# yahoo/TensorFlowOnSpark

Measured on AMD Instinct MI355X. Metric: images/sec (whole node) ResNet-50 sync-SGD InputMode.SPARK, higher is better.
Workload: dtype bf16; 1 GPU; model=resnet50, global_batch=1024, per_gpu_batch=1024, parallelism=dp1

## Files before the change

### csrc/bindings.cpp

```cpp
#include <torch/extension.h>
#include <c10/hip/HIPStream.h>
#include <hip/hip_runtime.h>
#include <climits>

extern "C" {
int tfosr_bn_fast_blocks(long, int, int, int);
void tfosr_bn_apply_dual(const void*, const void*, void*, unsigned char*,
                         const float*, const float*, const float*, const float*,
                         const float*, const float*, const float*, const float*,
                         int, long, int, hipStream_t);
void tfosr_bn_bwd_stats_dual(const void*, const void*, const void*,
                             const unsigned char*, const float*, const float*,
                             const float*, const float*, float*, int, int, long,
                             int, hipStream_t);
void tfosr_bn_bwd_merge_dual(const float*, int, float*, float*, float*, float*,
                             int, hipStream_t);
void tfosr_bn_bwd_dx_dual(const void*, const void*, const void*,
                          const unsigned char*, void*, void*, const float*,
                          const float*, const float*, const float*, const float*,
                          const float*, const float*, const float*, const float*,
                          int, long, int, hipStream_t);
void tfosr_bn_stats(const void*, int, int, float*, int, int, int, long, hipStream_t);
void tfosr_bn_finalize(const float*, int, const void*, int, int, long,
                       float*, float*, float*, float*,
                       long, int, float, float, hipStream_t);
void tfosr_bn_apply(const void*, const void*, void*, unsigned char*,
// ... 58 lines not shown
                           int, hipStream_t);
int tfosr_bn_tile_ws_rows(int);
void tfosr_bn_tile_finalize(const float*, int, int, float*, float*, float*,
                            float*, float*, long, int, float, float,
                            hipStream_t);
}

namespace tfosr {
uint32_t crc32c(const uint8_t*, size_t, uint32_t);
struct ScanResult {
  std::string buffer;
  std::vector<std::pair<size_t, size_t>> records;
};
ScanResult scan_file(const std::string&, bool);
void write_file(const std::string&, const std::vector<std::string>&, bool);
}

namespace {

hipStream_t cur_stream() {
  return c10::hip::getCurrentHIPStream().stream();
}

struct BNLayout {
  bool nhwc;
  int N, C;
  long HW;
};

BNLayout bn_layout(const at::Tensor& x) {
  TORCH_CHECK(x.dim() == 4, "expected 4-D NCHW tensor");
  BNLayout l;
  l.N = x.size(0);
  l.C = x.size(1);
  l.HW = (long)x.size(2) * x.size(3);
  if (x.is_contiguous(at::MemoryFormat::ChannelsLast)) {
    l.nhwc = true;
  } else {
    TORCH_CHECK(x.is_contiguous(), "input must be contiguous (NCHW or channels_last)");
    l.nhwc = false;
  }
  return l;
}

int dtype_flag(const at::Tensor& x) {
  TORCH_CHECK(x.is_cuda(), "bn: input must be a GPU tensor");
// ... 794 lines not shown
              "conv_mfma: filter dilation fd > 1 requires input dilation "
              "D == 1");
  TORCH_CHECK(fd <= kMaxTapReach && fd * (fh - 1) <= kMaxTapReach &&
                  fd * (fw - 1) <= kMaxTapReach,
              "conv_mfma: fd, fd*(fh-1) and fd*(fw-1) must be <= ",
              kMaxTapReach);
  long taps = fh * fw;
  int N = x.size(0), Cin = x.size(1), H = x.size(2), W = x.size(3);
  TORCH_CHECK(Cin % 32 == 0, "conv_mfma requires Cin % 32 == 0");
  TORCH_CHECK(wk.size(1) == taps * Cin);
  if (OH < 0) {
    long HV = (H - 1) * D + 1, WV = (W - 1) * D + 1;
    long nh = HV + 2 * P - fd * (fh - 1) - 1;
    long nw = WV + 2 * P - fd * (fw - 1) - 1;
    TORCH_CHECK(nh >= 0 && nw >= 0,
                "conv_mfma: the dilated filter does not fit the padded "
                "input");
    OH = nh / S + 1;
    OW = nw / S + 1;
  }
  auto y = at::empty({N, Cout, OH, OW},
                     x.options().dtype(out_f32 ? at::kFloat : at::kBFloat16),
                     at::MemoryFormat::ChannelsLast);
  auto guard = at::zeros({64}, x.options());
  if (stats && D == 1 && !out_f32) {
    TORCH_CHECK(x.is_cuda() && wk.device() == x.device(),
                "conv_mfma_stats: x and wk must be on one GPU");
    const long M = (long)N * OH * OW;
    auto part = at::empty({(M + 255) / 256, 2, Cout},
                          x.options().dtype(at::kFloat));
    tfosr_conv_mfma_stats(x.data_ptr(), wk.contiguous().data_ptr(),
                          guard.data_ptr(), y.data_ptr(),
                          part.data_ptr<float>(), N, H, W, Cin, Cout, OH, OW, S,
                          P, taps, fw, (int)fd, cur_stream());
    return {y, part};
  }
  tfosr_conv_mfma(x.data_ptr(), wk.contiguous().data_ptr(), guard.data_ptr(),
                  y.data_ptr(), out_f32 ? 0 : 1, N, H, W, Cin,
                  Cout, OH, OW, S, P, taps, fw, D, 0, (int)fd, cur_stream());
  return {y, c10::nullopt};
}

PYBIND11_MODULE(TORCH_EXTENSION_NAME, m) {
  m.def("api_version", []() { return TFOSR_API_VERSION; });
  m.def("bn_fwd_train", &bn_fwd_train);
  m.def("bn_fwd_eval", &bn_fwd_eval);
  m.def("bn_bwd", &bn_bwd);
  m.def("bn_dual_eligible", &bn_dual_eligible);
  m.def("bn_dual_fwd_train", &bn_dual_fwd_train);
  m.def("bn_dual_bwd", &bn_dual_bwd);
  m.def("bn_fast_blocks", [](long total, int C, bool bf16, bool nhwc) {
    return tfosr_bn_fast_blocks(total, C, bf16, nhwc);
  });
  m.def("bn_stage", &bn_stage);
  m.def("softmax_xent_fwd", &softmax_xent_fwd);
  m.def("softmax_xent_bwd", &softmax_xent_bwd);
  m.def("xent_dense_fwd", &xent_dense_fwd, py::arg("logits"), py::arg("target"),
        py::arg("ignore_index") = -100, py::arg("label_smoothing") = 0.0,
        py::arg("reduction") = 0, py::arg("max_grid") = 0);
  m.def("xent_dense_bwd", &xent_dense_bwd, py::arg("logits"), py::arg("lse"),
// ... 22 lines not shown
                                   x.size(2), x.size(3), K, S, P);
    int N = x.size(0), C = x.size(1), H = x.size(2), W = x.size(3);
    int OH = (int)ohw.first, OW = (int)ohw.second;
    auto y = at::empty({N, C, OH, OW}, x.options(),
                       at::MemoryFormat::ChannelsLast);
    auto idx = at::empty({N, OH, OW, C}, x.options().dtype(at::kByte));
    tfosr_maxpool_fwd(x.data_ptr(), y.data_ptr(), idx.data_ptr<unsigned char>(),
                      x.scalar_type() == at::kBFloat16, N, C, H, W, OH, OW,
                      K, S, P, cur_stream());
    return std::vector<at::Tensor>{y, idx};
  });
  m.def("conv3x3_fwd", [](at::Tensor x, at::Tensor w9, long Cout, long S,
                          long P) {
    TORCH_CHECK(x.dim() == 4 && x.is_contiguous(at::MemoryFormat::ChannelsLast),
                "conv3x3_fwd expects channels_last input");
    TORCH_CHECK(x.scalar_type() == at::kBFloat16 &&
                w9.scalar_type() == at::kBFloat16);
    int N = x.size(0), Cin = x.size(1), H = x.size(2), W = x.size(3);
    TORCH_CHECK(Cin % 32 == 0, "conv3x3 requires Cin % 32 == 0");
    TORCH_CHECK(w9.size(1) == 9 * Cin);
    int OH = (H + 2 * P - 3) / S + 1, OW = (W + 2 * P - 3) / S + 1;
    auto y = at::empty({N, Cout, OH, OW}, x.options(),
                       at::MemoryFormat::ChannelsLast);
    auto guard = at::zeros({64}, x.options());
    tfosr_conv3x3(x.data_ptr(), w9.contiguous().data_ptr(), guard.data_ptr(),
                  y.data_ptr(), 1, N, H, W, Cin, Cout, OH, OW,
                  S, P, cur_stream());
    return y;
  });
  m.def("conv_mfma", [](at::Tensor x, at::Tensor wk, long Cout, long fh,
                        long fw, long S, long P, long D, long OH, long OW,
                        long fd, bool out_f32) {
    return conv_mfma_impl(x, wk, Cout, fh, fw, S, P, D, OH, OW, fd, out_f32,
                          false).first;
  }, py::arg("x"), py::arg("wk"), py::arg("Cout"), py::arg("fh"),
     py::arg("fw"), py::arg("S"), py::arg("P"), py::arg("D"), py::arg("OH"),
     py::arg("OW"), py::arg("fd") = 1, py::arg("out_f32") = false);
  m.def("conv_mfma_stats", [](at::Tensor x, at::Tensor wk, long Cout, long fh,
                              long fw, long S, long P, long D, long OH,
                              long OW, long fd, bool out_f32) {
    auto r = conv_mfma_impl(x, wk, Cout, fh, fw, S, P, D, OH, OW, fd, out_f32,
                            true);
    if (!r.second.has_value()) return py::make_tuple(r.first, py::none(), 0);
    return py::make_tuple(r.first, *r.second, 256);
  }, py::arg("x"), py::arg("wk"), py::arg("Cout"), py::arg("fh"),
     py::arg("fw"), py::arg("S"), py::arg("P"), py::arg("D"), py::arg("OH"),
     py::arg("OW"), py::arg("fd") = 1, py::arg("out_f32") = false);
  m.def("gemm_bt_stats", &gemm_bt_stats, py::arg("a"), py::arg("b"));
  m.def("bn_fwd_train_pre", &bn_fwd_train_pre);
  m.def("bn_dual_fwd_train_pre", &bn_dual_fwd_train_pre);
  m.def("bn_batch_stats", &bn_batch_stats);
  m.def("conv_mfma_acc", [](at::Tensor x, at::Tensor wk, at::Tensor out,
                            long fh, long fw, long S, long P, long D) {
    TORCH_CHECK(x.is_contiguous(at::MemoryFormat::ChannelsLast) &&
                out.is_contiguous(at::MemoryFormat::ChannelsLast));
    TORCH_CHECK(x.scalar_type() == at::kBFloat16 &&
                wk.scalar_type() == at::kBFloat16 &&
                out.scalar_type() == at::kBFloat16);
    int N = x.size(0), Cin = x.size(1), H = x.size(2), W = x.size(3);
    TORCH_CHECK(Cin % 32 == 0, "conv_mfma requires Cin % 32 == 0");
    long taps = fh * fw;
    TORCH_CHECK(wk.size(1) == taps * Cin);
    long Cout = out.size(1), OH = out.size(2), OW = out.size(3);
    TORCH_CHECK(out.size(0) == N);
    auto guard = at::zeros({64}, x.options());
    tfosr_conv_mfma(x.data_ptr(), wk.contiguous().data_ptr(), guard.data_ptr(),
                    out.data_ptr(), 1, N, H, W, Cin, Cout, OH, OW,
                    S, P, taps, fw, D, 1, 1, cur_stream());
    return out;
  });
  m.def("gemm_bt_acc", [](at::Tensor a, at::Tensor b, at::Tensor c) {
    TORCH_CHECK(a.dim() == 2 && b.dim() == 2 && c.dim() == 2,
                "gemm_bt_acc: A[M,K], B[N,K], C[M,N] must be 2-D");
    TORCH_CHECK(a.is_cuda(), "gemm_bt_acc: a must be a GPU tensor");
    TORCH_CHECK(b.device() == a.device() && c.device() == a.device(),
                "gemm_bt_acc: b and c must be on ", a.device());
    TORCH_CHECK(a.is_contiguous() && b.is_contiguous() && c.is_contiguous(),
                "gemm_bt_acc: a, b and c must be contiguous");
    TORCH_CHECK(a.scalar_type() == at::kBFloat16 &&
                    b.scalar_type() == at::kBFloat16 &&
                    c.scalar_type() == at::kBFloat16,
                "gemm_bt_acc: a, b and c must be bfloat16");
    long M = a.size(0), K = a.size(1), Nn = b.size(0);
    TORCH_CHECK(b.size(1) == K && c.size(0) == M && c.size(1) == Nn,
                "gemm_bt_acc: A[M,K], B[N,K], C[M,N]");
    TORCH_CHECK(K % 32 == 0, "gemm_bt_acc: K must be a multiple of 32");
    tfosr_gemm_bt_acc(a.data_ptr(), b.data_ptr(), c.data_ptr(),
                      1, M, Nn, K, 1, cur_stream());
    return c;
// ... 1 lines not shown
  m.def("conv_wrw2", [](at::Tensor dy, at::Tensor x, long R, long S_f,
                        long stride, long P, long fd) {
    TORCH_CHECK(dy.is_contiguous(at::MemoryFormat::ChannelsLast) &&
                x.is_contiguous(at::MemoryFormat::ChannelsLast));
    TORCH_CHECK(dy.scalar_type() == at::kBFloat16 &&
                x.scalar_type() == at::kBFloat16);
    int N = x.size(0), Cin = x.size(1), H = x.size(2), W = x.size(3);
    int Cout = dy.size(1), OH = dy.size(2), OW = dy.size(3);
    TORCH_CHECK(Cin % 8 == 0 && Cout % 8 == 0,
                "conv_wrw2 needs channel counts % 8 == 0");
    long taps = R * S_f;
    TORCH_CHECK(taps == 1 || taps == 9, "conv_wrw2 supports 1x1 and 3x3");
    TORCH_CHECK(fd >= 1, "conv_wrw2: filter dilation fd must be >= 1, got ",
                fd);
    TORCH_CHECK(taps != 1 || fd == 1,
                "conv_wrw2: a 1x1 filter has no dilation, fd must be 1");
    TORCH_CHECK(fd <= kMaxTapReach && fd * (R - 1) <= kMaxTapReach &&
                    fd * (S_f - 1) <= kMaxTapReach,
                "conv_wrw2: fd, fd*(R-1) and fd*(S_f-1) must be <= ",
                kMaxTapReach);
    long M = (long)N * OH * OW;
    int split = tfosr_wrw2_split(Cout, Cin, M);
    long K = taps * (long)Cin;
    auto ws = at::empty({(long)split, (long)Cout * K},
                        x.options().dtype(at::kFloat));
    auto dW = at::empty({(long)Cout, K}, x.options().dtype(at::kFloat));
    auto guard = at::zeros({64}, x.options());
    tfosr_conv_wrw2(dy.data_ptr(), x.data_ptr(), guard.data_ptr(),
                    ws.data_ptr<float>(), dW.data_ptr<float>(), N, H, W, Cin,
                    Cout, OH, OW, R, S_f, stride, P, split, (int)fd,
                    cur_stream());
    return dW;
  }, py::arg("dy"), py::arg("x"), py::arg("R"), py::arg("S_f"),
     py::arg("stride"), py::arg("P"), py::arg("fd") = 1);
  m.def("pack_bf16", [](at::Tensor descs, at::Tensor cum, long ndesc,
                        at::Tensor arena, long total) {
    TORCH_CHECK(descs.is_cuda() && cum.is_cuda() && arena.is_cuda() &&
                    descs.device() == arena.device() &&
                    cum.device() == arena.device(),
                "pack_bf16 expects descs, cum and arena on one GPU");
    TORCH_CHECK(arena.scalar_type() == at::kBFloat16 && arena.is_contiguous(),
                "pack_bf16 expects a contiguous bf16 arena");
    TORCH_CHECK(ndesc >= 0 && ndesc <= INT_MAX, "pack_bf16: bad ndesc ", ndesc);
    TORCH_CHECK(descs.scalar_type() == at::kByte && descs.is_contiguous() &&
                    descs.numel() == ndesc * 80,
                "pack_bf16: descs must hold ndesc * 80 contiguous bytes");
    TORCH_CHECK(cum.scalar_type() == at::kLong && cum.is_contiguous() &&
                    cum.numel() == ndesc + 1,
                "pack_bf16: cum must hold ndesc + 1 contiguous int64");
    TORCH_CHECK(total >= 0 && arena.numel() >= total,
                "pack_bf16: arena holds ", arena.numel(), " elements, total is ",
// ... 4 lines not shown
                    arena.data_ptr(), total, cur_stream());
  });
  m.def("conv_par", [](at::Tensor x, at::Tensor wk, at::Tensor out,
                       std::vector<long> taps_r, std::vector<long> taps_s,
                       long P, bool accum) {
    TORCH_CHECK(x.is_contiguous(at::MemoryFormat::ChannelsLast) &&
                out.is_contiguous(at::MemoryFormat::ChannelsLast));
    TORCH_CHECK(x.scalar_type() == at::kBFloat16 &&
                wk.scalar_type() == at::kBFloat16 &&
                out.scalar_type() == at::kBFloat16);
    int N = x.size(0), Cin = x.size(1), H = x.size(2), W = x.size(3);
    TORCH_CHECK(Cin % 32 == 0);
    long ntaps = (long)taps_r.size();
    TORCH_CHECK(ntaps >= 1 && ntaps <= 8 && taps_s.size() == (size_t)ntaps);
    TORCH_CHECK(wk.size(1) == ntaps * Cin);
    long Cout = out.size(1), OHr = out.size(2), OWr = out.size(3);
    long oh0 = ((P - taps_r[0]) % 2 + 2) % 2;
    long ow0 = ((P - taps_s[0]) % 2 + 2) % 2;
    long OHs = (OHr - oh0 + 1) / 2, OWs = (OWr - ow0 + 1) / 2;
    if (OHs <= 0 || OWs <= 0) return out;
    unsigned long pack = 0;
    for (long i = 0; i < ntaps; ++i)
      pack |= ((unsigned long)((taps_r[i] << 4) | taps_s[i])) << (i * 8);
    auto guard = at::zeros({64}, x.options());
    tfosr_conv_par(x.data_ptr(), wk.contiguous().data_ptr(), guard.data_ptr(),
                   out.data_ptr(), N, H, W, Cin, (int)Cout, (int)OHs,
                   (int)OWs, (int)P, (int)ntaps, pack, (int)oh0, (int)ow0,
                   (int)OWr, OHr * OWr, accum ? 1 : 0, cur_stream());
    return out;
  });
  m.def("conv_stem", [](at::Tensor x4, at::Tensor w224, long Cout) {
    TORCH_CHECK(x4.is_contiguous(at::MemoryFormat::ChannelsLast) &&
                x4.size(1) == 4, "conv_stem expects NHWC4 padded input");
    TORCH_CHECK(x4.scalar_type() == at::kBFloat16 &&
                w224.scalar_type() == at::kBFloat16);
    TORCH_CHECK(w224.size(1) == 224);
    int N = x4.size(0), Hp = x4.size(2), Wp = x4.size(3);
    int OH = (Hp - 7) / 2 + 1, OW = (Wp - 7) / 2 + 1;
    auto y = at::empty({N, Cout, OH, OW}, x4.options(),
                       at::MemoryFormat::ChannelsLast);
    auto guard = at::zeros({64}, x4.options());
    tfosr_conv_stem(x4.data_ptr(), w224.contiguous().data_ptr(),
                    guard.data_ptr(), y.data_ptr(), N, Hp, Wp, Cout, OH, OW,
                    cur_stream());
    return y;
  });
  m.def("conv_stem_wrw", [](at::Tensor dy, at::Tensor x4) {
    TORCH_CHECK(dy.is_contiguous(at::MemoryFormat::ChannelsLast) &&
                x4.is_contiguous(at::MemoryFormat::ChannelsLast));
    TORCH_CHECK(dy.scalar_type() == at::kBFloat16 &&
                x4.scalar_type() == at::kBFloat16 && x4.size(1) == 4);
    int N = x4.size(0), Hp = x4.size(2), Wp = x4.size(3);
    int Cout = dy.size(1), OH = dy.size(2), OW = dy.size(3);
    long M = (long)N * OH * OW;
    int split = tfosr_wrw2_split(Cout, 32, M);
    long K = 7L * 32;
    auto ws = at::empty({(long)split, (long)Cout * K},
                        x4.options().dtype(at::kFloat));
    auto dW = at::empty({(long)Cout, K}, x4.options().dtype(at::kFloat));
    auto guard = at::zeros({64}, x4.options());
    tfosr_conv_wrw2(dy.data_ptr(), x4.data_ptr(), guard.data_ptr(),
                    ws.data_ptr<float>(), dW.data_ptr<float>(), N, Hp, Wp,
                    32, Cout, OH, OW, 7, 1,
                    2, 0, split, 1, cur_stream());
    return dW;
  });
  m.def("conv_wrw", [](at::Tensor dy, at::Tensor x, long R, long S, long P) {
    TORCH_CHECK(dy.is_contiguous(at::MemoryFormat::ChannelsLast) &&
                x.is_contiguous(at::MemoryFormat::ChannelsLast));
    TORCH_CHECK(dy.scalar_type() == at::kBFloat16 &&
                x.scalar_type() == at::kBFloat16);
    int N = x.size(0), Cin = x.size(1), H = x.size(2), W = x.size(3);
    int Cout = dy.size(1), OH = dy.size(2), OW = dy.size(3);
    auto dW = at::zeros({Cout, R * S * (long)Cin},
                        x.options().dtype(at::kFloat));
    tfosr_conv_wrw(dy.data_ptr(), x.data_ptr(), dW.data_ptr<float>(), N, H, W,
                   Cin, Cout, OH, OW, R, S, P, cur_stream());
    return dW;
  });
  m.def("maxpool_bwd", [](at::Tensor dy, at::Tensor idx, long H, long W,
                          long K, long S, long P) {
    TORCH_CHECK(dy.dim() == 4, "maxpool_bwd expects a 4-D gradient");
    auto ohw = check_pool_geometry("maxpool_bwd", dy, dy.size(1), dy.size(0),
                                   H, W, K, S, P);
// ... 37 lines not shown
```

### csrc/conv_wrw2.hip

```cpp
#include "tfosr_common.h"

typedef short s16x4 __attribute__((ext_vector_type(4)));
typedef short bf16x8 __attribute__((ext_vector_type(8)));
typedef float f32x4 __attribute__((ext_vector_type(4)));

#define AS3 __attribute__((address_space(3)))

__device__ __forceinline__ void wrw_stage16(const char* src, AS3 char* dst) {
  __builtin_amdgcn_global_load_lds(
      (const __attribute__((address_space(1))) void*)src, (AS3 void*)dst, 16,
      0, 0);
}

__device__ __forceinline__ unsigned wrw_div(unsigned m, unsigned long magic) {
  return (unsigned)(((unsigned long)m * magic) >> 40);
}

template <int TAPS, int DEPTH>
__global__ __launch_bounds__(256, 1) void conv_wrw2_kernel(
    const bf16_t* __restrict__ dy, const bf16_t* __restrict__ X,
    const bf16_t* __restrict__ guard, float* __restrict__ ws,
    int Nn, int H, int W, int Cin, int Cout, int OH, int OW, int FW,
    int stride, int P, int pixst, int steps_per_wg, long M,
    unsigned long magicOW, unsigned long magicOHOW, int ntn, int split,
    int fd) {
  constexpr int REG = TAPS + 1;
  constexpr int REGB = 32 * 64 * 2;
  constexpr int SLOT = REG * REGB;
  constexpr int CPT = REG * 256 / 256;
  __shared__ char lds[DEPTH * SLOT];
  AS3 char* lds3 = (AS3 char*)lds;

  const int nwg = gridDim.x;
  int wgid = blockIdx.x;
  {
    const int q = nwg / 8, r = nwg % 8;
    const int xcd = wgid % 8, pos = wgid / 8;
    wgid = (xcd < r ? xcd * (q + 1) : r * (q + 1) + (xcd - r) * q) + pos;
  }
  const int tile = wgid / split;
  const int sp = wgid - tile * split;
  const int cout0 = (tile / ntn) * 64;
  const int cin0 = (tile % ntn) * 64;

  const long m_begin = (long)sp * steps_per_wg * 32;
  const int t = threadIdx.x;
  const int lane = t & 63;
  const int wc = t >> 6;

  const int mloc = (t >> 1) & 31;
  int ch_isdy[CPT], ch_r[CPT], ch_s[CPT], ch_ldsoff[CPT];
  long ch_coff[CPT];
  #pragma unroll
  for (int u = 0; u < CPT; ++u) {
    int q = t + u * 256;
    int region = q >> 8;
    int cb = (q >> 6) & 3, h = (q & 1) ^ ((q >> 4) & 1);
    int tap = region - 1;
    ch_isdy[u] = region == 0;
    ch_r[u] = region ? (tap / FW) * fd - P : 0;
    ch_s[u] = region ? (tap % FW) * fd - P : 0;
    ch_ldsoff[u] = q * 16;
    int cglob = (region == 0 ? cout0 : cin0) + cb * 16 + h * 8;
    int climit = region == 0 ? Cout : Cin;
    ch_coff[u] = (cglob + 7 < climit) ? (long)cglob * 2 : -1;
  }

  unsigned invmask[DEPTH];
  auto stage = [&](int slot, long m0) {
    AS3 char* base = lds3 + slot * SLOT;
    long m = m0 + mloc;
    const bool mok = m < M;
    unsigned mm = (unsigned)(mok ? m : 0);
    unsigned n = wrw_div(mm, magicOHOW);
    unsigned rem = mm - n * (unsigned)(OH * OW);
    unsigned oh = wrw_div(rem, magicOW);
    unsigned ow = rem - oh * (unsigned)OW;
    const int ohS = (int)oh * stride, owS = (int)ow * stride;
    const char* dyrow = (const char*)dy + mm * (long)Cout * 2;
    const char* xbase = (const char*)X + (long)n * H * W * (long)pixst * 2;
// ... 6 lines not shown
      int ihc = inimg ? ih : 0, iwc = inimg ? iw : 0;
      long coff = ch_coff[u] >= 0 ? ch_coff[u] : 0;
      const char* real = ch_isdy[u] ? dyrow + coff
                                    : xbase + ihc * rowb + iwc * colb + coff;
      if (!(mok && ch_coff[u] >= 0 && (ch_isdy[u] || inimg)))
        inv |= 1u << u;
      wrw_stage16(real, base + ch_ldsoff[u]);
    }
    invmask[slot] = inv;
  };
  auto zero_invalid = [&](int slot) {
    unsigned inv = invmask[slot];
    if (inv) {
      AS3 char* zb = lds3 + slot * SLOT;
      #pragma unroll
      for (int u = 0; u < CPT; ++u)
        if (inv & (1u << u)) {
          typedef int i32x4 __attribute__((ext_vector_type(4)));
          *(AS3 i32x4*)(zb + ch_ldsoff[u]) = (i32x4){0, 0, 0, 0};
        }
    }
  };

  f32x4 acc[4][TAPS];
  #pragma unroll
  for (int i = 0; i < 4; ++i)
    #pragma unroll
    for (int j = 0; j < TAPS; ++j) acc[i][j] = {0.f, 0.f, 0.f, 0.f};

  long nkt = (M - m_begin + 31) / 32;
  if (nkt > steps_per_wg) nkt = steps_per_wg;
  if (nkt <= 0) nkt = 0;

  const int lbase =
      ((((lane >> 4) * 8 + ((lane & 15) >> 2)) * 16) +
       ((lane & 3) ^ (((lane >> 4) & 1) << 1)) * 4) * 2;

  auto trread8 = [&](AS3 char* region, int blk) -> bf16x8 {
    AS3 s16x4* p =
        (AS3 s16x4*)(region + blk * 1024 + lbase);
    s16x4 lo = __builtin_amdgcn_ds_read_tr16_b64_v4i16(p);
    s16x4 hi = __builtin_amdgcn_ds_read_tr16_b64_v4i16(
        (AS3 s16x4*)((AS3 char*)p + 128));
    bf16x8 f;
    f[0] = lo[0]; f[1] = lo[1]; f[2] = lo[2]; f[3] = lo[3];
    f[4] = hi[0]; f[5] = hi[1]; f[6] = hi[2]; f[7] = hi[3];
    return f;
  };

  #pragma unroll
  for (int pf = 0; pf < DEPTH - 1; ++pf)
    if (pf < nkt) stage(pf, m_begin + (long)pf * 32);
  constexpr int INFLIGHT = (DEPTH - 1) * CPT;

  for (long kt = 0; kt < nkt; ++kt) {
    if (kt + DEPTH - 1 < nkt) {
      stage((int)((kt + DEPTH - 1) % DEPTH), m_begin + (kt + DEPTH - 1) * 32);
      asm volatile("s_waitcnt vmcnt(%0)" ::"i"(INFLIGHT) : "memory");
    } else {
      asm volatile("s_waitcnt vmcnt(0)" ::: "memory");
    }
    zero_invalid((int)(kt % DEPTH));
    asm volatile("s_waitcnt lgkmcnt(0)" ::: "memory");
    __builtin_amdgcn_sched_barrier(0);
    __syncthreads();

    AS3 char* slot = lds3 + (kt % DEPTH) * SLOT;
    bf16x8 afrag[4], bfrag[TAPS];
    #pragma unroll
    for (int co = 0; co < 4; ++co)
      afrag[co] = trread8(slot, co);
    #pragma unroll
    for (int tap = 0; tap < TAPS; ++tap)
      bfrag[tap] = trread8(slot + (tap + 1) * REGB, wc);
    __builtin_amdgcn_s_setprio(1);
    #pragma unroll
    for (int tap = 0; tap < TAPS; ++tap)
      #pragma unroll
      for (int co = 0; co < 4; ++co)
        acc[co][tap] = __builtin_amdgcn_mfma_f32_16x16x32_bf16(
            afrag[co], bfrag[tap], acc[co][tap], 0, 0, 0);
    __builtin_amdgcn_s_setprio(0);
    asm volatile("s_waitcnt lgkmcnt(0)" ::: "memory");
    __syncthreads();
  }

  const long K = (long)TAPS * Cin;
  float* out = ws + (long)sp * Cout * K;
  const int ccol = lane & 15;
  const int crow0 = (lane >> 4) * 4;
  const int cin_g = cin0 + wc * 16 + ccol;
  if (cin_g < Cin) {
    #pragma unroll
    for (int co = 0; co < 4; ++co) {
      int cout_g0 = cout0 + co * 16 + crow0;
      #pragma unroll
      for (int r = 0; r < 4; ++r) {
        int cout_g = cout_g0 + r;
        if (cout_g >= Cout) continue;
        #pragma unroll
        for (int tap = 0; tap < TAPS; ++tap)
          out[(long)cout_g * K + (long)tap * Cin + cin_g] = acc[co][tap][r];
      }
    }
  }
}


template <int DEPTH>
__global__ __launch_bounds__(256, 1) void wrw_gemm_tn_kernel(
    const bf16_t* __restrict__ dy, const bf16_t* __restrict__ X,
    const bf16_t* __restrict__ guard, float* __restrict__ ws,
    int Nn, int H, int W, int Cin, int Cout, int OH, int OW,
    int stride, int steps_per_wg, long M,
    unsigned long magicOW, unsigned long magicOHOW, int ntn, int split) {
  constexpr int REGB = 64 * 128 * 2;
  constexpr int SLOT = 2 * REGB;
  constexpr int CPT = 8;
// ... 140 lines not shown
    asm volatile("s_waitcnt lgkmcnt(0)" ::: "memory");
    __syncthreads();
  }

  float* out = ws + (long)sp * Cout * Cin;
  const int ccol = lane & 15;
  const int crow0 = (lane >> 4) * 4;
  #pragma unroll
  for (int j = 0; j < 4; ++j) {
    int cin_g = cin0 + wc * 64 + j * 16 + ccol;
    if (cin_g >= Cin) continue;
    #pragma unroll
    for (int i = 0; i < 4; ++i) {
      int cout_g0 = cout0 + wr * 64 + i * 16 + crow0;
      #pragma unroll
      for (int r = 0; r < 4; ++r) {
        if (cout_g0 + r >= Cout) continue;
        out[(long)(cout_g0 + r) * Cin + cin_g] = acc[i][j][r];
      }
    }
  }
}

__global__ void wrw_reduce_kernel(const float* __restrict__ ws,
                                  float* __restrict__ dW, long n, int split) {
  long i = (long)blockIdx.x * blockDim.x + threadIdx.x;
  if (i >= n) return;
  float acc = 0.f;
  for (int s = 0; s < split; ++s) acc += ws[(long)s * n + i];
  dW[i] = acc;
}

extern "C" {

int tfosr_wrw2_split(int Cout, int Cin, long M) {
  int ntiles = ((Cout + 63) / 64) * ((Cin + 63) / 64);
  int split = 1024 / ntiles;
  if (split < 1) split = 1;
  long steps = (M + 31) / 32;
  while ((long)split * 8 > steps && split > 1) split /= 2;
  return split;
}

void tfosr_conv_wrw2(const void* dy, const void* x, const void* guard,
                     float* ws, float* dW, int N, int H, int W, int Cin,
                     int Cout, int OH, int OW, int R, int S_f, int stride,
                     int P, int split, int fd, hipStream_t s) {
  const long M = (long)N * OH * OW;
  const int taps = R * S_f;
  const unsigned long magicOW = (1UL << 40) / (unsigned)OW + 1;
  const unsigned long magicOHOW = (1UL << 40) / (unsigned)(OH * OW) + 1;
  int ntn = (Cin + 63) / 64;
  int ntiles = ((Cout + 63) / 64) * ntn;
  long steps = (M + 31) / 32;
  if (taps == 1) {
    ntn = (Cin + 127) / 128;
    ntiles = ((Cout + 127) / 128) * ntn;
    steps = (M + 63) / 64;
  }
  const int spw = (int)((steps + split - 1) / split);
  dim3 grid(ntiles * split), block(256);
  if (taps == 9)
    hipLaunchKernelGGL((conv_wrw2_kernel<9, 2>), grid, block, 0, s,
                       (const bf16_t*)dy, (const bf16_t*)x,
                       (const bf16_t*)guard, ws, N, H, W, Cin, Cout, OH, OW,
                       S_f, stride, P, Cin, spw, M, magicOW, magicOHOW, ntn,
                       split, fd);
  else if (taps == 7)
    hipLaunchKernelGGL((conv_wrw2_kernel<7, 2>), grid, block, 0, s,
                       (const bf16_t*)dy, (const bf16_t*)x,
                       (const bf16_t*)guard, ws, N, H, W, Cin, Cout, OH, OW,
                       S_f, stride, P, 4, spw, M, magicOW, magicOHOW, ntn,
                       split, 1);
  else if (taps == 1)
    hipLaunchKernelGGL((wrw_gemm_tn_kernel<2>), grid, block, 0, s,
                       (const bf16_t*)dy, (const bf16_t*)x,
                       (const bf16_t*)guard, ws, N, H, W, Cin, Cout, OH, OW,
                       stride, spw, M, magicOW, magicOHOW, ntn, split);
  const long n = (long)Cout * taps * Cin;
  dim3 rg((n + 255) / 256), rb(256);
  hipLaunchKernelGGL(wrw_reduce_kernel, rg, rb, 0, s, ws, dW, n, split);
}

}
```

### tensorflowonspark_amd/ops/modules.py

```python

import os

import torch
import torch.nn as nn
import torch.nn.functional as F

from . import get_ext
from .packplan import (EagerPacks, _class_taps, flipped, im2col,
                       parity_class, rows, rows_t, stem_w224)


def _cl_bf16(t):
    return t.contiguous(memory_format=torch.channels_last).to(torch.bfloat16)


def as2d(t):
    return t.permute(0, 2, 3, 1).reshape(-1, t.shape[1])


def as4d(t2d, n, h, w):
    return t2d.view(n, h, w, -1).permute(0, 3, 1, 2)


def _use_wrw2(k, cin, cout, mode=None):
    if mode is None:
        mode = os.environ.get("TFOS_WRW", "auto")
    if mode == "mfma2":
        return True
    if mode in ("miopen", "mfma"):
        return False
    return k == 3 and cin <= 64 and cout <= 64


def _wrw_backend(mode, k, cin, cout, stride, fd=1, transposed=False,
                 round1=True):
    ch8 = cin % 8 == 0 and cout % 8 == 0
# ... 347 lines not shown

    def extra_repr(self):
        return "k={}, s={}, p={}".format(self.k, self.s, self.p)



class _Conv1x1S2Fn(torch.autograd.Function):

    @staticmethod
    def forward(ctx, x, weight):
        ext = get_ext(required=True)
        if x.dtype != torch.bfloat16:
            x = x.to(torch.bfloat16)
        y = ext.conv_mfma(x, rows(weight), weight.shape[0], 1, 1, 2, 0, 1,
                          -1, -1)
        ctx.save_for_backward(x, weight)
        return y

    @staticmethod
    def backward(ctx, dy):
        x, weight = ctx.saved_tensors
        Cout, Cin = weight.shape[0], weight.shape[1]
        dy = _cl_bf16(dy)
        dx = torch.zeros(x.shape, device=x.device, dtype=torch.bfloat16) \
            .contiguous(memory_format=torch.channels_last)
        _conv_parity(dy, rows_t(weight).view(Cin, 1, 1, Cout), dx, 1, 0)
        return dx, _weight_grad(dy, x, weight, 1, 2, 0)


class _Conv1x1Fn(torch.autograd.Function):

    @staticmethod
    def forward(ctx, x, weight):
        ext = get_ext(required=True)
        N, _, H, W = x.shape
        x2d = as2d(x)
        if x2d.dtype != torch.bfloat16:
            x2d = x2d.to(torch.bfloat16)
        w2d = rows(weight)
        y2d = ext.gemm_bt(x2d, w2d, True)
        ctx.save_for_backward(x2d, w2d, weight)
        return as4d(y2d, N, H, W)

    @staticmethod
    def backward(ctx, dy):
        ext = get_ext(required=True)
        x2d, w2d, weight = ctx.saved_tensors
        N, _, H, W = dy.shape
# ... 38 lines not shown


class _Conv3x3Fn(torch.autograd.Function):

    @staticmethod
    def forward(ctx, x, weight, stride):
        ext = get_ext(required=True)
        if x.dtype != torch.bfloat16:
            x = x.to(torch.bfloat16)
        y = ext.conv_mfma(x, im2col(weight), weight.shape[0], 3, 3, stride,
                          1, 1, -1, -1)
        ctx.save_for_backward(x, weight)
        ctx.stride = stride
        return y

    @staticmethod
    def backward(ctx, dy):
        x, weight = ctx.saved_tensors
        S = ctx.stride
        Cout, Cin = weight.shape[0], weight.shape[1]
        dy = _cl_bf16(dy)
        wperm = flipped(weight)
        if S == 2:
            dx = torch.empty(x.shape, device=x.device, dtype=torch.bfloat16) \
                .contiguous(memory_format=torch.channels_last)
            _conv_parity(dy, wperm, dx, 3, 1)
        else:
            dx = get_ext(required=True).conv_mfma(
                dy, wperm.reshape(Cin, 9 * Cout), Cin, 3, 3, 1, 1, 1,
                x.shape[2], x.shape[3])
        return dx, _weight_grad(dy, x, weight, 3, S, 1), None


class Conv3x3(nn.Module):

    def __init__(self, cin, cout, stride=1):
        super().__init__()
        self.stride = stride
        self.weight = nn.Parameter(torch.empty(cout, cin, 3, 3))
        nn.init.kaiming_normal_(self.weight, mode="fan_out", nonlinearity="relu")
        self._eligible = cin % 32 == 0 and cout % 32 == 0 and cout >= 64 \
            and stride in (1, 2)

    def forward(self, x):
        backend = os.environ.get("TFOS_CONV3X3", "mfma")
        if x.is_cuda and self._eligible and backend == "mfma" \
                and x.dtype == torch.bfloat16 \
                and get_ext(required=True) is not None:
# ... 154 lines not shown
    return _parity_launch(
        x, lambda ph, pw, rl, sl: packs["{}_{}{}".format(prefix, ph, pw)],
        out, k, pp, accum)


def _conv_parity(x, wperm, out, k, pp, accum=False):
    return _parity_launch(
        x, lambda ph, pw, rl, sl: parity_class(wperm, rl, sl),
        out, k, pp, accum)



class _ConvT2dFn(torch.autograd.Function):

    @staticmethod
    def forward(ctx, x, weight, stride, padding, output_padding):
        _, Cout, KH, KW = weight.shape
        if x.dtype != torch.bfloat16:
            x = x.to(torch.bfloat16)
        wperm = flipped(weight)
        H, W = x.shape[2], x.shape[3]
        OH = (H - 1) * stride - 2 * padding + KH + output_padding
        OW = (W - 1) * stride - 2 * padding + KW + output_padding
        y = torch.empty(x.shape[0], Cout, OH, OW, device=x.device,
                        dtype=torch.bfloat16) \
            .contiguous(memory_format=torch.channels_last)
        if KH % 2 or output_padding:
            y.zero_()
        _conv_parity(x, wperm, y, KH, KH - 1 - padding)
        ctx.save_for_backward(x, weight)
        ctx.params = (stride, padding)
        return y

    @staticmethod
    def backward(ctx, dy):
        ext = get_ext(required=True)
        x, weight = ctx.saved_tensors
        S, P = ctx.params
        Cin, _, KH, KW = weight.shape
        dy = _cl_bf16(dy)
        dx = ext.conv_mfma(dy, im2col(weight), Cin, KH, KW, S, P, 1,
                           x.shape[2], x.shape[3])
        dw = _weight_grad(dy, x, weight, KH, S, P, transposed=True)
        return dx, dw, None, None, None


class ConvTranspose2dMFMA(nn.Module):

    def __init__(self, cin, cout, kernel_size=4, stride=2, padding=1,
# ... 286 lines not shown
        def cl(t):
            return t.contiguous(memory_format=torch.channels_last)

        def wrw(dyt, xt, w, k, s_):
            return _weight_grad(dyt, xt, w, k, s_, k // 2, round1=False)

        if dual:
            td, md, rd = opt
            dt3, dtd, dg3, dgd, db3, dbd = ext.bn_dual_bwd(
                t3, td, dy, k3, g3, m3, r3, gd, md, rd)
        else:
            dt3, dg3, db3, dres = ext.bn_bwd(t3, dy, y, k3, g3, m3, r3,
                                             True, True)
        dt3 = cl(dt3)

        da2 = cl(as4d(ext.gemm_bt(as2d(dt3), packs["w3bT"].reshape(C2, C3),
                                  True), N, OH, OW))
        dw3 = wrw(dt3, a2, w3, 1, 1)

        dt2, dg2, db2 = ext.bn_bwd(t2, da2, a2, k2, g2, m2, r2, True, False)
        dt2 = cl(dt2)

        if stride == 2:
            da1 = torch.empty(N, C1, H, W, device=x.device,
                              dtype=torch.bfloat16) \
                .contiguous(memory_format=torch.channels_last)
            _conv_parity_packed(dt2, packs, "w9p", da1, 3, 1)
        else:
            da1 = ext.conv_mfma(dt2, packs["w9p"].reshape(C1, 9 * C2), C1,
                                3, 3, 1, 1, 1, H, W)
        dw2 = wrw(dt2, a1, w2, 3, stride)

        dt1, dg1, db1 = ext.bn_bwd(t1, da1, a1, k1, g1, m1, r1, True, False)
        dt1 = cl(dt1)

        dw1 = wrw(dt1, x, w1, 1, 1)

        w1bT = packs["w1bT"].reshape(Cin, C1)
        if has_down:
            if not dual:
                td, idn, md, rd = opt
                dtd, dgd, dbd = ext.bn_bwd(td, dres, idn,
                                           torch.empty(0, dtype=torch.uint8,
                                                       device=td.device),
                                           gd, md, rd, False, False)
            dtd = cl(dtd)
            dwd = wrw(dtd, x, wd, 1, stride)
            dx = cl(as4d(ext.gemm_bt(as2d(dt1), w1bT, True), N, H, W))
            wdbT = packs["wdbT"].reshape(Cin, C3)
            if stride == 1:
                ext.gemm_bt_acc(as2d(dtd), wdbT, as2d(dx))
            else:
                ext.conv_par(dtd, wdbT, dx, [0], [0], 0, True)
        else:
            dx = dres
            ext.gemm_bt_acc(as2d(dt1), w1bT, as2d(dx))
            dwd = dgd = dbd = None

        return (dx, dw1, dg1, db1, None, None, dw2, dg2, db2, None, None,
                dw3, dg3, db3, None, None, dwd, dgd, dbd, None, None,
                None, None, None, None)



class _StemConvFn(torch.autograd.Function):

    @staticmethod
    def forward(ctx, x, weight, w224=None):
        ext = get_ext(required=True)
        N, _, H, W = x.shape
        Cout = weight.shape[0]
        x4 = torch.zeros(N, 4, H + 6, W + 6, dtype=torch.bfloat16,
                         device=x.device) \
            .contiguous(memory_format=torch.channels_last)
        x4[:, :3, 3:H + 3, 3:W + 3] = x
        if w224 is None:
            w224 = stem_w224(weight)
        y = ext.conv_stem(x4, w224.reshape(Cout, 224).contiguous(), Cout)
        ctx.save_for_backward(x4, weight)
        return y

    @staticmethod
    def backward(ctx, dy):
        ext = get_ext(required=True)
        x4, weight = ctx.saved_tensors
        dw224 = ext.conv_stem_wrw(_cl_bf16(dy), x4)
        Cout = weight.shape[0]
        dw = dw224.view(Cout, 7, 8, 4)[:, :, :7, :3].permute(0, 3, 1, 2)
        return None, dw.contiguous().to(weight.dtype), None


class StemConv7x7(nn.Module):

    def __init__(self, cin=3, cout=64):
        super().__init__()
        assert cin == 3
        self.weight = nn.Parameter(torch.empty(cout, cin, 7, 7))
# ... 88 lines not shown
```

Measured before the change: 10340 images/sec.

## Cache conv zero guard, retile 7-tap weight grad, vectorize split reduction, allocate channels_last directly

Measured after the change: 10760 images/sec, median of 6. 1.04x the previous value.

```diff
diff --git a/csrc/bindings.cpp b/csrc/bindings.cpp
--- a/csrc/bindings.cpp
+++ b/csrc/bindings.cpp
@@ -1,7 +1,10 @@
 #include <torch/extension.h>
 #include <c10/hip/HIPStream.h>
 #include <hip/hip_runtime.h>
+#include <c10/hip/HIPException.h>
 #include <climits>
+#include <map>
+#include <mutex>
 
 extern "C" {
 int tfosr_bn_fast_blocks(long, int, int, int);
@@ -106,6 +109,34 @@
   return c10::hip::getCurrentHIPStream().stream();
 }
 
+const void* zero_guard(const at::Tensor& like) {
+  constexpr size_t kGuardBytes = 256;
+  static std::mutex mu;
+  static std::map<int, void*> cache;
+  TORCH_CHECK(like.is_cuda(), "zero_guard: expected a GPU tensor");
+  const int dev = like.get_device();
+  std::lock_guard<std::mutex> lock(mu);
+  auto it = cache.find(dev);
+  if (it != cache.end()) return it->second;
+  hipStreamCaptureStatus cap = hipStreamCaptureStatusNone;
+  C10_HIP_CHECK(hipStreamIsCapturing(cur_stream(), &cap));
+  TORCH_CHECK(cap == hipStreamCaptureStatusNone,
+              "the conv kernels' zero guard for device ", dev,
+              " is created on first use with a blocking fill, which a stream "
+              "capture does not allow: run one conv on this device before "
+              "capturing");
+  int prev = 0;
+  C10_HIP_CHECK(hipGetDevice(&prev));
+  C10_HIP_CHECK(hipSetDevice(dev));
+  void* p = nullptr;
+  C10_HIP_CHECK(hipMalloc(&p, kGuardBytes));
+  C10_HIP_CHECK(hipMemset(p, 0, kGuardBytes));
+  C10_HIP_CHECK(hipDeviceSynchronize());
+  C10_HIP_CHECK(hipSetDevice(prev));
+  cache.emplace(dev, p);
+  return p;
+}
+
 struct BNLayout {
   bool nhwc;
   int N, C;
@@ -946,7 +977,7 @@
   auto y = at::empty({N, Cout, OH, OW},
                      x.options().dtype(out_f32 ? at::kFloat : at::kBFloat16),
                      at::MemoryFormat::ChannelsLast);
-  auto guard = at::zeros({64}, x.options());
+  const void* guard = zero_guard(x);
   if (stats && D == 1 && !out_f32) {
     TORCH_CHECK(x.is_cuda() && wk.device() == x.device(),
                 "conv_mfma_stats: x and wk must be on one GPU");
@@ -954,12 +985,12 @@
     auto part = at::empty({(M + 255) / 256, 2, Cout},
                           x.options().dtype(at::kFloat));
     tfosr_conv_mfma_stats(x.data_ptr(), wk.contiguous().data_ptr(),
-                          guard.data_ptr(), y.data_ptr(),
+                          guard, y.data_ptr(),
                           part.data_ptr<float>(), N, H, W, Cin, Cout, OH, OW, S,
                           P, taps, fw, (int)fd, cur_stream());
     return {y, part};
   }
-  tfosr_conv_mfma(x.data_ptr(), wk.contiguous().data_ptr(), guard.data_ptr(),
+  tfosr_conv_mfma(x.data_ptr(), wk.contiguous().data_ptr(), guard,
                   y.data_ptr(), out_f32 ? 0 : 1, N, H, W, Cin,
                   Cout, OH, OW, S, P, taps, fw, D, 0, (int)fd, cur_stream());
   return {y, c10::nullopt};
@@ -1028,8 +1059,8 @@
     int OH = (H + 2 * P - 3) / S + 1, OW = (W + 2 * P - 3) / S + 1;
     auto y = at::empty({N, Cout, OH, OW}, x.options(),
                        at::MemoryFormat::ChannelsLast);
-    auto guard = at::zeros({64}, x.options());
-    tfosr_conv3x3(x.data_ptr(), w9.contiguous().data_ptr(), guard.data_ptr(),
+    const void* guard = zero_guard(x);
+    tfosr_conv3x3(x.data_ptr(), w9.contiguous().data_ptr(), guard,
                   y.data_ptr(), 1, N, H, W, Cin, Cout, OH, OW,
                   S, P, cur_stream());
     return y;
@@ -1069,8 +1100,8 @@
     TORCH_CHECK(wk.size(1) == taps * Cin);
     long Cout = out.size(1), OH = out.size(2), OW = out.size(3);
     TORCH_CHECK(out.size(0) == N);
-    auto guard = at::zeros({64}, x.options());
-    tfosr_conv_mfma(x.data_ptr(), wk.contiguous().data_ptr(), guard.data_ptr(),
+    const void* guard = zero_guard(x);
+    tfosr_conv_mfma(x.data_ptr(), wk.contiguous().data_ptr(), guard,
                     out.data_ptr(), 1, N, H, W, Cin, Cout, OH, OW,
                     S, P, taps, fw, D, 1, 1, cur_stream());
     return out;
@@ -1118,11 +1149,13 @@
     long M = (long)N * OH * OW;
     int split = tfosr_wrw2_split(Cout, Cin, M);
     long K = taps * (long)Cin;
+    TORCH_CHECK((long)split * Cout * K < (1L << 32),
+                "conv_wrw2: the split workspace exceeds 2^32 elements");
     auto ws = at::empty({(long)split, (long)Cout * K},
                         x.options().dtype(at::kFloat));
     auto dW = at::empty({(long)Cout, K}, x.options().dtype(at::kFloat));
-    auto guard = at::zeros({64}, x.options());
-    tfosr_conv_wrw2(dy.data_ptr(), x.data_ptr(), guard.data_ptr(),
+    const void* guard = zero_guard(x);
+    tfosr_conv_wrw2(dy.data_ptr(), x.data_ptr(), guard,
                     ws.data_ptr<float>(), dW.data_ptr<float>(), N, H, W, Cin,
                     Cout, OH, OW, R, S_f, stride, P, split, (int)fd,
                     cur_stream());
@@ -1173,8 +1206,8 @@
     unsigned long pack = 0;
     for (long i = 0; i < ntaps; ++i)
       pack |= ((unsigned long)((taps_r[i] << 4) | taps_s[i])) << (i * 8);
-    auto guard = at::zeros({64}, x.options());
-    tfosr_conv_par(x.data_ptr(), wk.contiguous().data_ptr(), guard.data_ptr(),
+    const void* guard = zero_guard(x);
+    tfosr_conv_par(x.data_ptr(), wk.contiguous().data_ptr(), guard,
                    out.data_ptr(), N, H, W, Cin, (int)Cout, (int)OHs,
                    (int)OWs, (int)P, (int)ntaps, pack, (int)oh0, (int)ow0,
                    (int)OWr, OHr * OWr, accum ? 1 : 0, cur_stream());
@@ -1190,9 +1223,9 @@
     int OH = (Hp - 7) / 2 + 1, OW = (Wp - 7) / 2 + 1;
     auto y = at::empty({N, Cout, OH, OW}, x4.options(),
                        at::MemoryFormat::ChannelsLast);
-    auto guard = at::zeros({64}, x4.options());
+    const void* guard = zero_guard(x4);
     tfosr_conv_stem(x4.data_ptr(), w224.contiguous().data_ptr(),
-                    guard.data_ptr(), y.data_ptr(), N, Hp, Wp, Cout, OH, OW,
+                    guard, y.data_ptr(), N, Hp, Wp, Cout, OH, OW,
                     cur_stream());
     return y;
   });
@@ -1206,11 +1239,13 @@
     long M = (long)N * OH * OW;
     int split = tfosr_wrw2_split(Cout, 32, M);
     long K = 7L * 32;
+    TORCH_CHECK((long)split * Cout * K < (1L << 32),
+                "conv_stem_wrw: the split workspace exceeds 2^32 elements");
     auto ws = at::empty({(long)split, (long)Cout * K},
                         x4.options().dtype(at::kFloat));
     auto dW = at::empty({(long)Cout, K}, x4.options().dtype(at::kFloat));
-    auto guard = at::zeros({64}, x4.options());
-    tfosr_conv_wrw2(dy.data_ptr(), x4.data_ptr(), guard.data_ptr(),
+    const void* guard = zero_guard(x4);
+    tfosr_conv_wrw2(dy.data_ptr(), x4.data_ptr(), guard,
                     ws.data_ptr<float>(), dW.data_ptr<float>(), N, Hp, Wp,
                     32, Cout, OH, OW, 7, 1,
                     2, 0, split, 1, cur_stream());
diff --git a/csrc/conv_wrw2.hip b/csrc/conv_wrw2.hip
--- a/csrc/conv_wrw2.hip
+++ b/csrc/conv_wrw2.hip
@@ -16,7 +16,7 @@
   return (unsigned)(((unsigned long)m * magic) >> 40);
 }
 
-template <int TAPS, int DEPTH>
+template <int TAPS, int DEPTH, int CIN_T = 64>
 __global__ __launch_bounds__(256, 1) void conv_wrw2_kernel(
     const bf16_t* __restrict__ dy, const bf16_t* __restrict__ X,
     const bf16_t* __restrict__ guard, float* __restrict__ ws,
@@ -24,10 +24,17 @@
     int stride, int P, int pixst, int steps_per_wg, long M,
     unsigned long magicOW, unsigned long magicOHOW, int ntn, int split,
     int fd) {
-  constexpr int REG = TAPS + 1;
-  constexpr int REGB = 32 * 64 * 2;
-  constexpr int SLOT = REG * REGB;
-  constexpr int CPT = REG * 256 / 256;
+  static_assert(CIN_T == 64 || CIN_T == 32, "x tile is 64 or 32 channels");
+  constexpr int MSTEP = CIN_T == 64 ? 32 : 64;
+  constexpr int MH = MSTEP / 32;
+  constexpr int BLKB = MSTEP * 16 * 2;
+  constexpr int DYCH = MSTEP * 8;
+  constexpr int XCH = MSTEP * CIN_T / 8;
+  constexpr int REGB_DY = DYCH * 16, REGB_X = XCH * 16;
+  constexpr int SLOT = REGB_DY + TAPS * REGB_X;
+  static_assert((DYCH + TAPS * XCH) % 256 == 0, "whole rounds of 256 chunks");
+  constexpr int CPT = (DYCH + TAPS * XCH) / 256;
+  constexpr int NCO = CIN_T == 64 ? 4 : 2;
   __shared__ char lds[DEPTH * SLOT];
   AS3 char* lds3 = (AS3 char*)lds;
 
@@ -41,21 +48,23 @@
   const int tile = wgid / split;
   const int sp = wgid - tile * split;
   const int cout0 = (tile / ntn) * 64;
-  const int cin0 = (tile % ntn) * 64;
-
-  const long m_begin = (long)sp * steps_per_wg * 32;
+  const int cin0 = (tile % ntn) * CIN_T;
+
+  const long m_begin = (long)sp * steps_per_wg * MSTEP;
   const int t = threadIdx.x;
   const int lane = t & 63;
-  const int wc = t >> 6;
-
-  const int mloc = (t >> 1) & 31;
+  const int wc = CIN_T == 64 ? t >> 6 : (t >> 6) & 1;
+  const int co0 = CIN_T == 64 ? 0 : (t >> 7) * NCO;
+
+  const int mloc = (t >> 1) & (MSTEP - 1);
   int ch_isdy[CPT], ch_r[CPT], ch_s[CPT], ch_ldsoff[CPT];
   long ch_coff[CPT];
   #pragma unroll
   for (int u = 0; u < CPT; ++u) {
     int q = t + u * 256;
-    int region = q >> 8;
-    int cb = (q >> 6) & 3, h = (q & 1) ^ ((q >> 4) & 1);
+    int region = q < DYCH ? 0 : 1 + (q - DYCH) / XCH;
+    int qq = q < DYCH ? q : (q - DYCH) % XCH;
+    int cb = qq / (MSTEP * 2), h = (q & 1) ^ ((q >> 4) & 1);
     int tap = region - 1;
     ch_isdy[u] = region == 0;
     ch_r[u] = region ? (tap / FW) * fd - P : 0;
@@ -108,13 +117,13 @@
     }
   };
 
-  f32x4 acc[4][TAPS];
-  #pragma unroll
-  for (int i = 0; i < 4; ++i)
+  f32x4 acc[NCO][TAPS];
+  #pragma unroll
+  for (int i = 0; i < NCO; ++i)
     #pragma unroll
     for (int j = 0; j < TAPS; ++j) acc[i][j] = {0.f, 0.f, 0.f, 0.f};
 
-  long nkt = (M - m_begin + 31) / 32;
+  long nkt = (M - m_begin + MSTEP - 1) / MSTEP;
   if (nkt > steps_per_wg) nkt = steps_per_wg;
   if (nkt <= 0) nkt = 0;
 
@@ -122,9 +131,9 @@
       ((((lane >> 4) * 8 + ((lane & 15) >> 2)) * 16) +
        ((lane & 3) ^ (((lane >> 4) & 1) << 1)) * 4) * 2;
 
-  auto trread8 = [&](AS3 char* region, int blk) -> bf16x8 {
+  auto trread8 = [&](AS3 char* region, int blk, int mh) -> bf16x8 {
     AS3 s16x4* p =
-        (AS3 s16x4*)(region + blk * 1024 + lbase);
+        (AS3 s16x4*)(region + blk * BLKB + mh * 1024 + lbase);
     s16x4 lo = __builtin_amdgcn_ds_read_tr16_b64_v4i16(p);
     s16x4 hi = __builtin_amdgcn_ds_read_tr16_b64_v4i16(
         (AS3 s16x4*)((AS3 char*)p + 128));
@@ -136,12 +145,13 @@
 
   #pragma unroll
   for (int pf = 0; pf < DEPTH - 1; ++pf)
-    if (pf < nkt) stage(pf, m_begin + (long)pf * 32);
+    if (pf < nkt) stage(pf, m_begin + (long)pf * MSTEP);
   constexpr int INFLIGHT = (DEPTH - 1) * CPT;
 
   for (long kt = 0; kt < nkt; ++kt) {
     if (kt + DEPTH - 1 < nkt) {
-      stage((int)((kt + DEPTH - 1) % DEPTH), m_begin + (kt + DEPTH - 1) * 32);
+      stage((int)((kt + DEPTH - 1) % DEPTH),
+            m_begin + (kt + DEPTH - 1) * MSTEP);
       asm volatile("s_waitcnt vmcnt(%0)" ::"i"(INFLIGHT) : "memory");
     } else {
       asm volatile("s_waitcnt vmcnt(0)" ::: "memory");
@@ -152,21 +162,24 @@
     __syncthreads();
 
     AS3 char* slot = lds3 + (kt % DEPTH) * SLOT;
-    bf16x8 afrag[4], bfrag[TAPS];
-    #pragma unroll
-    for (int co = 0; co < 4; ++co)
-      afrag[co] = trread8(slot, co);
-    #pragma unroll
-    for (int tap = 0; tap < TAPS; ++tap)
-      bfrag[tap] = trread8(slot + (tap + 1) * REGB, wc);
-    __builtin_amdgcn_s_setprio(1);
-    #pragma unroll
-    for (int tap = 0; tap < TAPS; ++tap)
-      #pragma unroll
-      for (int co = 0; co < 4; ++co)
-        acc[co][tap] = __builtin_amdgcn_mfma_f32_16x16x32_bf16(
-            afrag[co], bfrag[tap], acc[co][tap], 0, 0, 0);
-    __builtin_amdgcn_s_setprio(0);
+    #pragma unroll
+    for (int mh = 0; mh < MH; ++mh) {
+      bf16x8 afrag[NCO], bfrag[TAPS];
+      #pragma unroll
+      for (int co = 0; co < NCO; ++co)
+        afrag[co] = trread8(slot, co0 + co, mh);
+      #pragma unroll
+      for (int tap = 0; tap < TAPS; ++tap)
+        bfrag[tap] = trread8(slot + REGB_DY + tap * REGB_X, wc, mh);
+      __builtin_amdgcn_s_setprio(1);
+      #pragma unroll
+      for (int tap = 0; tap < TAPS; ++tap)
+        #pragma unroll
+        for (int co = 0; co < NCO; ++co)
+          acc[co][tap] = __builtin_amdgcn_mfma_f32_16x16x32_bf16(
+              afrag[co], bfrag[tap], acc[co][tap], 0, 0, 0);
+      __builtin_amdgcn_s_setprio(0);
+    }
     asm volatile("s_waitcnt lgkmcnt(0)" ::: "memory");
     __syncthreads();
   }
@@ -178,8 +191,8 @@
   const int cin_g = cin0 + wc * 16 + ccol;
   if (cin_g < Cin) {
     #pragma unroll
-    for (int co = 0; co < 4; ++co) {
-      int cout_g0 = cout0 + co * 16 + crow0;
+    for (int co = 0; co < NCO; ++co) {
+      int cout_g0 = cout0 + (co0 + co) * 16 + crow0;
       #pragma unroll
       for (int r = 0; r < 4; ++r) {
         int cout_g = cout_g0 + r;
@@ -366,13 +379,61 @@
   }
 }
 
-__global__ void wrw_reduce_kernel(const float* __restrict__ ws,
-                                  float* __restrict__ dW, long n, int split) {
-  long i = (long)blockIdx.x * blockDim.x + threadIdx.x;
-  if (i >= n) return;
-  float acc = 0.f;
-  for (int s = 0; s < split; ++s) acc += ws[(long)s * n + i];
-  dW[i] = acc;
+constexpr int RED_COLS = 64, RED_GROUPS = 4, RED_U = 4, RED_CHUNK = 64;
+
+template <int VEC>
+__global__ __launch_bounds__(RED_COLS * RED_GROUPS) void wrw_reduce_kernel(
+    const float* src, float* dst, unsigned ncol, int rows, int chunk,
+    unsigned src_row, unsigned dst_row) {
+  typedef float vec_t __attribute__((ext_vector_type(VEC)));
+  __shared__ vec_t part[RED_GROUPS - 1][RED_COLS];
+  const int lane = threadIdx.x & (RED_COLS - 1);
+  const int g = threadIdx.x / RED_COLS;
+  const unsigned col = blockIdx.x * RED_COLS + lane;
+  const bool live = col < ncol;
+  const int s0 = blockIdx.y * chunk;
+  const int s1 = min(s0 + chunk, rows);
+  const vec_t zero = {};
+  vec_t acc = zero;
+  if (live) {
+    const vec_t* p = (const vec_t*)src + col;
+    for (int s = s0 + g; s < s1; s += RED_GROUPS * RED_U) {
+      vec_t v[RED_U];
+      #pragma unroll
+      for (int u = 0; u < RED_U; ++u) {
+        const int su = s + u * RED_GROUPS;
+        v[u] = su < s1 ? p[(unsigned)su * (src_row / VEC)] : zero;
+      }
+      #pragma unroll
+      for (int u = 0; u < RED_U; ++u) acc += v[u];
+    }
+  }
+  if (g > 0) part[g - 1][lane] = acc;
+  __syncthreads();
+  if (g == 0 && live) {
+    #pragma unroll
+    for (int k = 0; k < RED_GROUPS - 1; ++k) acc += part[k][lane];
+    ((vec_t*)dst)[blockIdx.y * (dst_row / VEC) + col] = acc;
+  }
+}
+
+template <int VEC>
+static void wrw_reduce_launch(float* ws, float* dW, long n, int split,
+                              hipStream_t s) {
+  const unsigned ncol = (unsigned)(n / VEC);
+  const unsigned cb = (ncol + RED_COLS - 1) / RED_COLS;
+  dim3 block(RED_COLS * RED_GROUPS);
+  if (split <= RED_CHUNK) {
+    hipLaunchKernelGGL((wrw_reduce_kernel<VEC>), dim3(cb, 1), block, 0, s, ws,
+                       dW, ncol, split, split, (unsigned)n, 0u);
+    return;
+  }
+  const int nchunk = (split + RED_CHUNK - 1) / RED_CHUNK;
+  hipLaunchKernelGGL((wrw_reduce_kernel<VEC>), dim3(cb, nchunk), block, 0, s,
+                     ws, ws, ncol, split, RED_CHUNK, (unsigned)n,
+                     (unsigned)(RED_CHUNK * n));
+  hipLaunchKernelGGL((wrw_reduce_kernel<VEC>), dim3(cb, 1), block, 0, s, ws,
+                     dW, ncol, nchunk, nchunk, (unsigned)(RED_CHUNK * n), 0u);
 }
 
 extern "C" {
@@ -401,6 +462,10 @@
     ntn = (Cin + 127) / 128;
     ntiles = ((Cout + 127) / 128) * ntn;
     steps = (M + 63) / 64;
+  } else if (taps == 7) {
+    ntn = (Cin + 31) / 32;
+    ntiles = ((Cout + 63) / 64) * ntn;
+    steps = (M + 63) / 64;
   }
   const int spw = (int)((steps + split - 1) / split);
   dim3 grid(ntiles * split), block(256);
@@ -411,7 +476,7 @@
                        S_f, stride, P, Cin, spw, M, magicOW, magicOHOW, ntn,
                        split, fd);
   else if (taps == 7)
-    hipLaunchKernelGGL((conv_wrw2_kernel<7, 2>), grid, block, 0, s,
+    hipLaunchKernelGGL((conv_wrw2_kernel<7, 2, 32>), grid, block, 0, s,
                        (const bf16_t*)dy, (const bf16_t*)x,
                        (const bf16_t*)guard, ws, N, H, W, Cin, Cout, OH, OW,
                        S_f, stride, P, 4, spw, M, magicOW, magicOHOW, ntn,
@@ -422,8 +487,10 @@
                        (const bf16_t*)guard, ws, N, H, W, Cin, Cout, OH, OW,
                        stride, spw, M, magicOW, magicOHOW, ntn, split);
   const long n = (long)Cout * taps * Cin;
-  dim3 rg((n + 255) / 256), rb(256);
-  hipLaunchKernelGGL(wrw_reduce_kernel, rg, rb, 0, s, ws, dW, n, split);
-}
-
-}
+  if (n % 4 == 0)
+    wrw_reduce_launch<4>(ws, dW, n, split, s);
+  else
+    wrw_reduce_launch<1>(ws, dW, n, split, s);
+}
+
+}
diff --git a/tensorflowonspark_amd/ops/modules.py b/tensorflowonspark_amd/ops/modules.py
--- a/tensorflowonspark_amd/ops/modules.py
+++ b/tensorflowonspark_amd/ops/modules.py
@@ -12,6 +12,15 @@
 
 def _cl_bf16(t):
     return t.contiguous(memory_format=torch.channels_last).to(torch.bfloat16)
+
+
+def _cl_alloc(shape, device, dtype=torch.bfloat16, zero=False):
+    shape = tuple(shape)
+    nchw_is_cl = len(shape) == 4 and (shape[1] == 1 or shape[2:] == (1, 1))
+    t = torch.empty(shape, device=device, dtype=dtype,
+                    memory_format=torch.contiguous_format if nchw_is_cl
+                    else torch.channels_last)
+    return t.zero_() if zero else t
 
 
 def as2d(t):
@@ -405,8 +414,7 @@
         x, weight = ctx.saved_tensors
         Cout, Cin = weight.shape[0], weight.shape[1]
         dy = _cl_bf16(dy)
-        dx = torch.zeros(x.shape, device=x.device, dtype=torch.bfloat16) \
-            .contiguous(memory_format=torch.channels_last)
+        dx = _cl_alloc(x.shape, x.device, zero=True)
         _conv_parity(dy, rows_t(weight).view(Cin, 1, 1, Cout), dx, 1, 0)
         return dx, _weight_grad(dy, x, weight, 1, 2, 0)
 
@@ -491,8 +499,7 @@
         dy = _cl_bf16(dy)
         wperm = flipped(weight)
         if S == 2:
-            dx = torch.empty(x.shape, device=x.device, dtype=torch.bfloat16) \
-                .contiguous(memory_format=torch.channels_last)
+            dx = _cl_alloc(x.shape, x.device)
             _conv_parity(dy, wperm, dx, 3, 1)
         else:
             dx = get_ext(required=True).conv_mfma(
@@ -693,9 +700,7 @@
         H, W = x.shape[2], x.shape[3]
         OH = (H - 1) * stride - 2 * padding + KH + output_padding
         OW = (W - 1) * stride - 2 * padding + KW + output_padding
-        y = torch.empty(x.shape[0], Cout, OH, OW, device=x.device,
-                        dtype=torch.bfloat16) \
-            .contiguous(memory_format=torch.channels_last)
+        y = _cl_alloc((x.shape[0], Cout, OH, OW), x.device)
         if KH % 2 or output_padding:
             y.zero_()
         _conv_parity(x, wperm, y, KH, KH - 1 - padding)
@@ -1028,9 +1033,7 @@
         dt2 = cl(dt2)
 
         if stride == 2:
-            da1 = torch.empty(N, C1, H, W, device=x.device,
-                              dtype=torch.bfloat16) \
-                .contiguous(memory_format=torch.channels_last)
+            da1 = _cl_alloc((N, C1, H, W), x.device)
             _conv_parity_packed(dt2, packs, "w9p", da1, 3, 1)
         else:
             da1 = ext.conv_mfma(dt2, packs["w9p"].reshape(C1, 9 * C2), C1,
@@ -1076,9 +1079,7 @@
         ext = get_ext(required=True)
         N, _, H, W = x.shape
         Cout = weight.shape[0]
-        x4 = torch.zeros(N, 4, H + 6, W + 6, dtype=torch.bfloat16,
-                         device=x.device) \
-            .contiguous(memory_format=torch.channels_last)
+        x4 = _cl_alloc((N, 4, H + 6, W + 6), x.device, zero=True)
         x4[:, :3, 3:H + 3, 3:W + 3] = x
         if w224 is None:
             w224 = stem_w224(weight)
```
